# anhtu293/nndepth

Measured on AMD Instinct MI355X. Metric: stereo pairs/sec at 544x960, 32 iters (RAFT-Stereo), higher is better.
Workload: dtype f32 carried as 2 range-scaled fp16 pieces per operand (3 MFMA products, fp32 accumulate); 1 GPU; RAFT-Stereo base (ctx 64), 544x960, 32 iters, batch 1 per GPU, all 32 up_disp emitted; parallelism=single, launch=direct

## Files before the change

### nndepth_amd/csrc/common.h

```cpp
#pragma once
#include <hip/hip_runtime.h>
#include <atomic>
#include <cstdarg>
#include <cstdio>
#include "../../include/nndepth_amd.h"
#include "split_arith.h"

namespace nnd {

void set_error(const char* fmt, ...);

#define NND_HIP_CHECK(expr)                                                              \
    do {                                                                                 \
        hipError_t _e = (expr);                                                          \
        if (_e != hipSuccess) {                                                          \
            nnd::set_error("%s failed: %s (%s:%d)", #expr, hipGetErrorString(_e), __FILE__, __LINE__); \
            return NND_ERR_HIP;                                                          \
        }                                                                                \
    } while (0)

#define NND_LAUNCH_CHECK()                                                               \
    do {                                                                                 \
        hipError_t _e = hipGetLastError();                                               \
        if (_e != hipSuccess) {                                                          \
// ... 9 lines not shown
            return NND_ERR_INVALID;                                                      \
        }                                                                                \
    } while (0)

#define NND_TRY(x)                           \
    do {                                     \
        if ((rc = (x)) != NND_OK) return rc; \
    } while (0)

template <class Desc>
static inline int check_desc(const Desc* d, unsigned allowed_flags, const char* name) {
    NND_REQUIRE(d, "%s: null descriptor", name);
    NND_REQUIRE(d->struct_size == (int32_t)sizeof(Desc), "%s: descriptor of %d bytes, this library expects %d (struct_size)", name,
                d->struct_size, (int)sizeof(Desc));
    NND_REQUIRE((d->flags & ~allowed_flags) == 0, "%s: unknown flags 0x%x", name, d->flags);
    return NND_OK;
}

struct Switches {
    bool no_fused_upsample, no_fused_lookup, no_fused_flow_branch, no_c4, agcl_v1, no_thin3d, corr_build_v1, corr_build_no_ksplit, igev_squeeze_v1, igev_squeeze_walk, no_folded_flow_head, no_conv1x1_stream,
        conv_verbose, debug_sync;
    int split_ny, split_ks, split_p;
    bool split_no_fast;
    bool no_merged_fb_lookup;
    int conv_p, conv_ks, conv_wco;
    int agcl_pb;
    bool lds_poison_on;
    unsigned lds_poison;
    int lds_slack;
    bool enc_no_c4;
    bool no_slab3d;
    int slab3d_rounds;
    bool no_fused_enc_block;
};
const Switches& switches();

static inline int raise_lds_limit(const void* kern, std::atomic<unsigned>& done, int bytes = 160 * 1024) {
    int dev = 0;
    NND_HIP_CHECK(hipGetDevice(&dev));
    const unsigned bit = 1u << (dev & 31);
    if (!(done.load(std::memory_order_relaxed) & bit)) {
        NND_HIP_CHECK(hipFuncSetAttribute(kern, hipFuncAttributeMaxDynamicSharedMemorySize, bytes));
        done.fetch_or(bit, std::memory_order_relaxed);
    }
    return NND_OK;
}

bool calibrating();
struct CalibScope {
    explicit CalibScope(bool on);
    ~CalibScope();
    CalibScope(const CalibScope&) = delete;
    CalibScope& operator=(const CalibScope&) = delete;
    bool on;
};
struct Act;
struct Lay;
int calib_amax_act(const Act& a, const Lay& lay, int B, int H, int W, const float* tail, hipStream_t s);
int calib_amax_flat(const float* x, int64_t n, const float* tail, hipStream_t s);
int calib_finish(float* blob, const int64_t* tail_offs, int n, int32_t* status_dev, hipStream_t s);

#ifdef __HIPCC__
__device__ __forceinline__ void fmac_scalar(float& acc, float a, float b) { asm("v_fmac_f32 %0, %1, %2" : "+v"(acc) : "v"(a), "v"(b)); }

__device__ __forceinline__ float relu_nan(float v) { return __builtin_elementwise_maximum(v, 0.f); }
__device__ __forceinline__ float clamp_nan(float v, float lo, float hi) {
// ... 42 lines not shown
    int64_t bstride;
    int C;
};

struct ConvIO {
    Act src0, src1;
    Act out0, out1;
    Act aux0, aux1;
    Act bmap;
    int hidden = 0;
    float scale = 1.f;
    int Hin = 0, Win = 0;
    int flags = 0;
    bool src_tiled = false;
    bool dst_tiled = false;
    bool src_c4 = false;
    bool dst_c4 = false;
    int cout_need = 0;
    int force_ks = 0;
};

static inline bool conv_shape_built(int KH, int KW) { return (KH == 1 && (KW == 1 || KW == 5)) || (KW == 1 && KH == 5) || (KH == 3 && KW == 3); }

int conv_ci_t(int KH, int KW, int Cin, int stride = 1, int Cout = 0);

int launch_conv(const ConvLayer& L, const float* blob, const ConvIO& io, int epi,
                int B, int H, int W, hipStream_t stream);

void pack_conv(const ConvLayer& L, int nparts, const float* const* w, const float* const* b,
               const int* cout, float* blob, const int* ci_map = nullptr, int cin_src = 0);

bool conv_split_supported(int KH, int KW, int Cin, int stride, int arith, int Cout = 0);
int launch_conv_split(const ConvLayer& L, const float* blob, const ConvIO& io, int epi, int B, int H, int W, hipStream_t stream);
bool conv_split_no_split_k(const ConvLayer& L, int B, int H, int W);
bool flow_branch_supported(const ConvLayer& f2, int fc);
int launch_flow_branch(const ConvLayer& f2, const float* blob, const float* w7t, const float* b7, const float* flow, int64_t fbs,
                       int fc, const ConvIO& io, int B, int H, int W, hipStream_t stream);
void pack_conv_split(const ConvLayer& L, int nparts, const float* const* w, const float* const* b, const int* cout, float* blob,
                     const int* ci_map, int cin_src);

bool enc_block_supported(const ConvLayer& c1, const ConvLayer& c2, const ConvLayer& ds);
int enc_block_launch(const ConvLayer& c1, const float* blob1, const ConvLayer& c2, const float* blob2, const ConvLayer& ds, const float* blobd,
                     const float* x, float* out, int N, int Hx, int Wx, hipStream_t stream);

bool thin3d_supported(int Cout, int stride);
bool slab3d_supported(int Cout, int C0, int C1, int stride, int arith);
int64_t slab3d_packed_floats(int Cout, int Ct, int stride);
void slab3d_pack(int Cout, int Ct, int stride, const float* w, const float* scale, const float* shift, float* out);
int slab3d_forward(int Cout, int C0, int C1, int stride, const float* packed, const float* x0, const float* x1, float* y, int N, int D,
                   int H, int W, float slope, hipStream_t s);
int64_t thin3d_packed_floats(int Cout, int Ct);
void thin3d_pack(int Cout, int Ct, const float* w, const float* scale, const float* shift, float* out);
int thin3d_forward(int Cout, int C0, int C1, int stride, const float* packed, const float* x0, const float* x1, float* y, int N, int D,
                   int H, int W, float slope, hipStream_t s);

int corr1d_lookup_launch(const float* pyr, const float* coords, float* out, int B, int H, int W, int num_levels,
                         int radius, hipStream_t stream, bool tiled);
int group_lookup_flat_launch(const float* pyr, const float* coords, float* out, int B, int G, int H, int W, int num_levels, int radius,
                             hipStream_t stream, bool tiled);
int igev_lookup_launch(const float* feat_pyramid, const float* geo_pyramid, const float* coords, float* out, int B, int G, int H,
                       int W, int num_levels, int radius, hipStream_t stream, bool tiled);
int convex_upsample_launch(const float* flow, const float* mask, float* out, int B, int C, int H, int W, int rate,
                           hipStream_t stream, bool tiled);

int agcl_iter_launch(const float* f1, const float* f2, const float* flow, float* warped, float* out, int N, int C, int H,
                     int W, int small_patch, hipStream_t s, bool tiled);
// ... 38 lines not shown
```

### nndepth_amd/csrc/conv_split.hip

```cpp
#include "conv_launch.h"
#include "conv_split_kernel.h"
#include "flow_branch.h"

#include <atomic>
#include <cmath>
#include <cstdlib>
#include <cstring>

namespace nnd {

namespace {
uint16_t f16_rn(float x) {
    const _Float16 h = (_Float16)x;
    uint16_t u;
    memcpy(&u, &h, 2);
    return u;
}
float f16_to_f(uint16_t u) {
    _Float16 h;
    memcpy(&h, &u, 2);
    return (float)h;
}
uint16_t bf16_rn(float x) {
    uint32_t u;
// ... 85 lines not shown

bool restrict_split(const ConvLayer& L, int cout_need, SplitCfg* cfg) {
    const int npos = split_patch(L.KH, L.KW, L.arith, L.stride).NPOS;
    auto units = [&](int wco) { return split_staging_units(cfg->P, npos, cfg->ks, wco * cfg->ks); };
    if (!conv_restrict_cout(L, cout_need, &cfg->ny, &cfg->wco, [&](int wco) { return cfg->P == 2 && units(wco) <= 4; })) return false;
    cfg->nu = split_nu_variant(units(cfg->wco));
    return true;
}

bool split_fast_ok(const ConvLayer& L) { return !switches().split_no_fast || L.stride == 2; }
bool plan_split(const ConvLayer& L, const ConvIO& io, int B, int H, int W, SplitCfg* cfg) {
    if (!pick_split(L, io.src0.C, io.src1.C, B, H, W, split_fast_ok(L), cfg)) return false;
    cfg->restricted = restrict_split(L, io.cout_need, cfg);
    cfg->grid = dim3(cdiv(cfg->ntiles, cfg->P), cfg->ny, B), cfg->block = dim3(64 * cfg->wco * cfg->ks);
    return true;
}

void print_split_plan(const ConvLayer& L, const ConvIO& io, const SplitCfg& cfg) {
    fprintf(stderr, "[nnd] conv_split %dx%d Cin=%d Cout=%d pieces=%d: ny=%d, wco=%d, ks=%d, P=%d, nu=%d%s, grid %ux%ux%u, lds %zu B%s%s\n", L.KH,
            L.KW, L.Cin, L.Cout, L.arith, cfg.ny, cfg.wco, cfg.ks, cfg.P, cfg.nu, cfg.fast ? ", fast" : "", cfg.grid.x, cfg.grid.y, cfg.grid.z, cfg.lds,
            io.cout_need > 0 ? (cfg.restricted ? ", restricted to the wanted output channels" : ", whole layer (not restrictable)") : "",
            L.stride == 2 ? ", stride 2" : "");
}
}

bool conv_split_no_split_k(const ConvLayer& L, int B, int H, int W) {
    SplitCfg cfg;
    return pick_split(L, L.Cin, 0, B, H, W, split_fast_ok(L), &cfg) && cfg.ks == 1;
}

extern template int launch_split_ns<1>(const ConvArgs&, const SplitCfg&, int, int, hipStream_t);
extern template int launch_split_ns<2>(const ConvArgs&, const SplitCfg&, int, int, hipStream_t);
extern template int launch_split_ns<3>(const ConvArgs&, const SplitCfg&, int, int, hipStream_t);

bool conv_split_supported(int KH, int KW, int Cin, int stride, int arith, int Cout) {
    if ((arith != 3 && arith != 2 && arith != 1) || (stride != 1 && stride != 2) || Cin % 16 != 0) return false;
    if (stride == 2) return ((KH == 3 && KW == 3) || (KH == 1 && KW == 1)) && Cout >= 96;
    return conv_shape_built(KH, KW);
}

int launch_conv_split(const ConvLayer& L, const float* blob, const ConvIO& io, int epi, int B, int H, int W, hipStream_t stream) {
    int rc, Hin, Win;
    NND_REQUIRE(conv_split_supported(L.KH, L.KW, L.Cin, L.stride, L.arith, L.Cout), "conv_split: %dx%d Cin=%d Cout=%d stride %d arith %d not built",
                L.KH, L.KW, L.Cin, L.Cout, L.stride, L.arith);
    NND_TRY(conv_check_io("conv_split", L, io, epi, H, W, &Hin, &Win));
    NND_REQUIRE(L.CI_T == 16 && L.nchunks * 16 == L.Cin, "conv_split: layer was not planned for 16-channel chunks");
    NND_REQUIRE(L.stride == 1 || io.src1.C == 0, "conv_split: stride 2 is built for one source");
    NND_REQUIRE((long)(L.Cin + 64) * tiled_plane(Hin, Win) < (1L << 31), "conv_split: plane offsets exceed 32 bits");
    SplitCfg cfg;
    NND_REQUIRE(plan_split(L, io, B, H, W, &cfg),
                "conv_split: no configuration for %dx%d Cin=%d (%d+%d) Cout=%d stride %d (NND_SPLIT_CFG ny=%d ks=%d P=%d%s)", L.KH, L.KW,
                L.Cin, io.src0.C, io.src1.C, L.Cout, L.stride, switches().split_ny, switches().split_ks, switches().split_p,
                split_fast_ok(L) ? "" : ", NND_SPLIT_NO_FAST");
    ConvArgs a;
    conv_fill_args(L, blob, io, epi, H, W, Hin, Win, &a);
    a.tiles_x = cfg.tiles_x; a.wco = cfg.wco; a.ks = cfg.ks; a.npos = cfg.ntiles;
#ifdef NND_DBG_STAMPS
    {
        static std::atomic<int> launches{0};
        static const int only = getenv("NND_DBG_STAMP_LAUNCH") ? atoi(getenv("NND_DBG_STAMP_LAUNCH")) : -1;
        const int idx = launches.fetch_add(1);
        a.dbg_stamp = only < 0 || idx == only;
    }
#endif
    if (calibrating() && split_range_scaled(L.arith))
        for (const Act* src : {&io.src0, &io.src1}) NND_TRY(calib_amax_act(*src, a.ls, B, Hin, Win, blob + L.tail_off(), stream));
    if (switches().conv_verbose) print_split_plan(L, io, cfg);
    rc = L.arith == 3   ? launch_split_ns<3>(a, cfg, L.KH, L.KW, stream)
         : L.arith == 2 ? launch_split_ns<2>(a, cfg, L.KH, L.KW, stream)
                        : launch_split_ns<1>(a, cfg, L.KH, L.KW, stream);
    NND_REQUIRE(rc != NND_ERR_UNSUPPORTED, "conv_split: shape %dx%d P=%d nu=%d %s is not instantiated", L.KH, L.KW, cfg.P, cfg.nu, cfg.fast ? "fast" : "generic");
    if (rc != NND_OK) return rc;
    NND_LAUNCH_CHECK();
    return NND_OK;
}

void pack_conv_split(const ConvLayer& L, int nparts, const float* const* w, const float* const* bvec, const int* cout, float* blob,
                     const int* ci_map, int cin_src) {
    if (!ci_map) cin_src = L.Cin;
    const int NT = L.KH * L.KW, NS = L.arith;
    uint16_t* wp = reinterpret_cast<uint16_t*>(blob + L.w_off);
    float* bp = blob + L.b_off;
    memset(wp, 0, sizeof(float) * L.w_floats());
    memset(bp, 0, sizeof(float) * L.b_floats());
    const bool f16 = split_range_scaled(NS);
    float wscale = 1.f;
    if (f16) {
        float wmax = 0.f;
        for (int part = 0; part < nparts; ++part)
            for (int col = 0; col < cout[part]; ++col)
                for (int ci = 0; ci < L.Cin; ++ci)
                    for (int t = 0; t < NT; ++t) {
                        const float v = std::fabs(w[part][((size_t)col * cin_src + (ci_map ? ci_map[ci] : ci)) * NT + t]);
                        if (std::isfinite(v) && v > wmax) wmax = v;
                    }
        int e = 0;
        if (wmax > 0.f) std::frexp(wmax, &e);
        const int s = wmax > 0.f ? 14 - e : 0;
        wscale = std::ldexp(1.f, s);
        float* tail = bp + L.ncb * 32;
        tail[SPLIT_TAIL_OSCALE] = std::ldexp(1.f, -(s + SPLIT_F16_XSHIFT));
        tail[SPLIT_TAIL_XSCALE] = std::ldexp(1.f, SPLIT_F16_XSHIFT);
        tail[SPLIT_TAIL_AMAX] = 0.f;
        tail[SPLIT_TAIL_WSINV] = std::ldexp(1.f, -s);
// ... 76 lines not shown
```

### nndepth_amd/csrc/conv_split_kernel.h

```cpp
#pragma once
#include "common.h"
#include "conv_epilogue.h"
#include "layout.h"
#include "split_arith.h"

#include <type_traits>
#include <utility>

namespace nnd {

#ifndef NND_SPLIT_BSLOTS
#define NND_SPLIT_BSLOTS 2
#endif

#ifdef NND_DBG_STAMPS
static __device__ unsigned long long g_split_stamps[4096 * 8];
#define NND_SSTAMP(i)                                                                                  \
    do {                                                                                               \
        if (threadIdx.x == 0 && a.dbg_stamp) {                                                         \
            const unsigned lin_ = blockIdx.x + gridDim.x * (blockIdx.y + gridDim.y * blockIdx.z);      \
            if (lin_ < 4096) g_split_stamps[lin_ * 8 + (i)] = __builtin_amdgcn_s_memrealtime();        \
        }                                                                                              \
    } while (0)
#define NND_SCLOCK(i)                                                                                  \
// ... 42 lines not shown
struct SplitPatch {
    int PRI, PCI, NPH, PRP, PCP, NPOS, PS, ROWB, PHB, SUBB;
};
__host__ __device__ constexpr SplitPatch split_patch(int KH, int KW, int NS, int STR) {
    const int PRI = 3 * STR + KH, PCI = 7 * STR + KW;
    const int NPH = STR == 1 ? 1 : (KH * KW == 1 ? 1 : 4);
    const int PRP = STR == 1 ? PRI : (KH == 1 ? 4 : (PRI + 1) / 2);
    const int PCP = STR == 1 ? PCI : (KW == 1 ? 8 : (PCI + 1) / 2);
    const int NPOS = STR == 1 ? PRI * PCI : (KH * KW == 1 ? 32 : PRI * PCI);
    const int ROWB = split_row_bytes(PCP, NS);
    return {PRI, PCI, NPH, PRP, PCP, NPOS, split_pos_bytes(NS), ROWB, PRP * ROWB, NPH * PRP * ROWB};
}
template <int KH, int KW, int NS, int STR>
struct SplitGeom {
    static constexpr SplitPatch G = split_patch(KH, KW, NS, STR);
    static constexpr int PRI = G.PRI, PCI = G.PCI, NPH = G.NPH, PRP = G.PRP, PCP = G.PCP, NPOS = G.NPOS;
    static constexpr int PS = G.PS, ROWB = G.ROWB, PHB = G.PHB, SUBB = G.SUBB;
};
__host__ __device__ constexpr int split_staging_units(int P, int npos, int ks, int waves) { return (P * npos * 2 * ks + 64 * waves - 1) / (64 * waves); }
__host__ __device__ constexpr int split_nu_variant(int nu) { return nu <= 2 ? 2 : 4; }

__host__ __device__ constexpr int split_pipe_spu(int nunit, int nsteps, int ul) {
    int v = 1;
    while (v < nsteps && nunit - 1 - (nsteps + v - 1) / v < ul + 3) ++v;
    return v;
}
template <int NT, int P, int NU>
struct SplitPipe {
    static constexpr int NUNIT = NT * P, NSTEPS = NU * 4 + 3, UL = 1;
    static constexpr int SPU = split_pipe_spu(NUNIT, NSTEPS, UL), U0 = NUNIT - 1 - (NSTEPS + SPU - 1) / SPU;
    static constexpr bool ON = NT >= 5 && P == 2;
};

template <int KH, int KW, int NS, int P, int NU, bool FAST, bool SRC4, int AD_, int MAXT, int STR = 1>
__global__ void __launch_bounds__(MAXT) conv_split_kernel(ConvArgs a) {
    static_assert(STR == 1 || (FAST && (KH * KW == 9 || KH * KW == 1)), "stride 2: 3x3 / 1x1, FAST regime");
    using Geo = SplitGeom<KH, KW, NS, STR>;
    constexpr int NT = KH * KW, PH = KH / 2, PW = KW / 2;
    constexpr int PC = Geo::PCI, NPOS = Geo::NPOS;
#ifndef NND_SPLIT_NO_PIPE
    constexpr bool PIPE = FAST && SRC4 && SplitPipe<NT, P, NU>::ON && NS != 1;
#else
    constexpr bool PIPE = false;
#endif
    constexpr int PS = Geo::PS, ROWB = Geo::ROWB, SUBB = Geo::SUBB, PHB = Geo::PHB;
    extern __shared__ __attribute__((aligned(16))) unsigned char lds_raw[];
    NND_SSTAMP(0);

    const int tid = threadIdx.x, lane = tid & 63, nthreads = blockDim.x;
    const int wave = __builtin_amdgcn_readfirstlane(tid >> 6);
    const int wco = a.wco, ks = a.ks;
    const int cbi = wave % wco, kj = wave / wco;
    const int h2 = lane >> 5, l31 = lane & 31;
    const int pxl = lane_pixel(l31), r = pxl >> 3, c = pxl & 7;
    const int cb = blockIdx.y * wco + cbi;
    const bool active = cb * 32 < a.Cout;
    const int b = blockIdx.z;
    const int Hin = a.Hin, Win = a.Win;
    const long SP = a.ls.plane;
    const int SCH = ks * 16;
    float oscale = 1.f, xscale = 1.f;
    if constexpr (split_range_scaled(NS)) {
        const float* tail = a.bias + (((a.Cout + 31) >> 5) << 5);
        oscale = tail[SPLIT_TAIL_OSCALE];
        xscale = tail[SPLIT_TAIL_XSCALE];
    }

    int ty0[P], tx0[P];
#pragma unroll
    for (int pp = 0; pp < P; ++pp) {
        const int t = blockIdx.x * P + pp;
        const bool valid = t < a.npos;
        ty0[pp] = valid ? (t / a.tiles_x) * 4 : (1 << 20);
        tx0[pp] = valid ? (t % a.tiles_x) * 8 : 0;
    }

    const int nunits = P * NPOS * 2 * ks;
    int goff[NU], loff[NU], cho[NU];
    bool inimg[NU], own[NU];
#pragma unroll
    for (int i = 0; i < NU; ++i) {
        const int u = PIPE ? min(tid + i * nthreads, nunits - 1) : tid + i * nthreads;
        own[i] = u < nunits;
        const int pos = u % NPOS, rest = u / NPOS;
        const int pp = rest % P, oct = rest / P;
        int pr, pc, lpos;
        if constexpr (STR == 1) {
            pr = pos / PC;
// ... 447 lines not shown
}

template <int KH, int KW, int NS, bool FAST, bool SRC4, int STR>
int launch_split_nu(const ConvArgs& a, const SplitCfg& cfg, hipStream_t stream) {
    constexpr int AD = FAST ? split_fast_ad<KH, KW, NS>() : 1;
    if (split_nu_variant(cfg.nu) == 2) return launch_split_kernel<KH, KW, NS, 2, 2, FAST, SRC4, AD, 768, STR>(a, cfg.grid, cfg.block, cfg.lds, stream);
    return launch_split_kernel<KH, KW, NS, 2, 4, FAST, SRC4, AD, 768, STR>(a, cfg.grid, cfg.block, cfg.lds, stream);
}
template <int KH, int KW, int NS>
int launch_split_shape(const ConvArgs& a, const SplitCfg& cfg, hipStream_t stream) {
    if (cfg.P != 2) return NND_ERR_UNSUPPORTED;
    const bool src4 = a.ls.ci == 4;
    if (cfg.stride == 2) {
        if constexpr (KH * KW == 9 || KH * KW == 1) {
            if (!cfg.fast) return NND_ERR_UNSUPPORTED;
            return src4 ? launch_split_nu<KH, KW, NS, true, true, 2>(a, cfg, stream) : launch_split_nu<KH, KW, NS, true, false, 2>(a, cfg, stream);
        } else {
            return NND_ERR_UNSUPPORTED;
        }
    }
    if (!cfg.fast) return launch_split_nu<KH, KW, NS, false, false, 1>(a, cfg, stream);
    return src4 ? launch_split_nu<KH, KW, NS, true, true, 1>(a, cfg, stream) : launch_split_nu<KH, KW, NS, true, false, 1>(a, cfg, stream);
}

template <int NS>
int launch_split_ns(const ConvArgs& a, const SplitCfg& cfg, int KH, int KW, hipStream_t stream) {
    if (KH == 3 && KW == 3) return launch_split_shape<3, 3, NS>(a, cfg, stream);
    if (KH == 1 && KW == 5) return launch_split_shape<1, 5, NS>(a, cfg, stream);
    if (KH == 5 && KW == 1) return launch_split_shape<5, 1, NS>(a, cfg, stream);
    if (KH == 1 && KW == 1) return launch_split_shape<1, 1, NS>(a, cfg, stream);
    return NND_ERR_UNSUPPORTED;
}

}
```

### nndepth_amd/csrc/conv_split_ns1.hip

```cpp
#include "conv_split_kernel.h"

namespace nnd {
template int launch_split_ns<1>(const ConvArgs&, const SplitCfg&, int, int, hipStream_t);
#ifdef NND_DBG_STAMPS
extern "C" int nnd_debug_read_split_stamps_ns1(unsigned long long* host, int n) {
    return hipMemcpyFromSymbol(host, HIP_SYMBOL(g_split_stamps), sizeof(unsigned long long) * n) == hipSuccess ? 0 : -1;
}
#endif
}
```

### nndepth_amd/csrc/conv_split_ns2.hip

```cpp
#include "conv_split_kernel.h"

namespace nnd {
template int launch_split_ns<2>(const ConvArgs&, const SplitCfg&, int, int, hipStream_t);
#ifdef NND_DBG_STAMPS
extern "C" int nnd_debug_read_split_stamps_ns2(unsigned long long* host, int n) {
    return hipMemcpyFromSymbol(host, HIP_SYMBOL(g_split_stamps), sizeof(unsigned long long) * n) == hipSuccess ? 0 : -1;
}
#endif
}
```

### nndepth_amd/csrc/conv_split_ns3.hip

```cpp
#include "conv_split_kernel.h"

namespace nnd {
template int launch_split_ns<3>(const ConvArgs&, const SplitCfg&, int, int, hipStream_t);
#ifdef NND_DBG_STAMPS
extern "C" int nnd_debug_read_split_stamps_ns3(unsigned long long* host, int n) {
    return hipMemcpyFromSymbol(host, HIP_SYMBOL(g_split_stamps), sizeof(unsigned long long) * n) == hipSuccess ? 0 : -1;
}
#endif
}
```

### nndepth_amd/csrc/error.cpp

```cpp
#include "common.h"

#include <cstdlib>

namespace nnd {
static thread_local char g_err[512] = "";
void set_error(const char* fmt, ...) {
    va_list ap;
    va_start(ap, fmt);
    vsnprintf(g_err, sizeof(g_err), fmt, ap);
    va_end(ap);
}

static Switches g_sw;
static void load_switches() {
    Switches s{};
    auto on = [](const char* n) { return getenv(n) != nullptr; };
    s.no_fused_upsample = on("NND_NO_FUSED_UPSAMPLE");
    s.no_fused_lookup = on("NND_NO_FUSED_LOOKUP");
    s.no_fused_flow_branch = on("NND_NO_FUSED_FLOW_BRANCH");
    s.no_c4 = on("NND_NO_C4");
    s.agcl_v1 = on("NND_AGCL_V1");
    s.no_thin3d = on("NND_NO_THIN3D");
    s.corr_build_v1 = on("NND_CORR_BUILD_V1");
    s.corr_build_no_ksplit = on("NND_CORR_BUILD_NO_KSPLIT");
    s.igev_squeeze_v1 = on("NND_IGEV_SQUEEZE_V1");
    s.igev_squeeze_walk = on("NND_IGEV_SQUEEZE_WALK");
    s.no_folded_flow_head = on("NND_NO_FOLDED_FLOW_HEAD");
    s.no_conv1x1_stream = on("NND_NO_CONV1X1_STREAM");
    s.conv_verbose = on("NND_CONV_VERBOSE");
    s.debug_sync = on("NND_DEBUG_SYNC");
    s.split_ny = s.split_ks = s.split_p = -1;
    if (const char* e = getenv("NND_SPLIT_CFG")) sscanf(e, "%d,%d,%d", &s.split_ny, &s.split_ks, &s.split_p);
    s.split_no_fast = on("NND_SPLIT_NO_FAST");
    s.no_merged_fb_lookup = on("NND_NO_MERGED_FB_LOOKUP");
    s.conv_p = s.conv_ks = s.conv_wco = -1;
    if (const char* e = getenv("NND_CONV_CFG")) sscanf(e, "%d,%d,%d", &s.conv_p, &s.conv_ks, &s.conv_wco);
    if (const char* e = getenv("NND_CONV_P")) s.conv_p = atoi(e);
    s.agcl_pb = getenv("NND_AGCL_PB") ? atoi(getenv("NND_AGCL_PB")) : 0;
    s.lds_poison_on = on("NND_DEBUG_LDS_POISON");
    s.lds_poison = s.lds_poison_on ? (unsigned)strtoul(getenv("NND_DEBUG_LDS_POISON"), nullptr, 0) : 0u;
    s.lds_slack = getenv("NND_DEBUG_LDS_SLACK") ? atoi(getenv("NND_DEBUG_LDS_SLACK")) : 0;
    s.enc_no_c4 = on("NND_ENC_NO_C4");
    s.no_slab3d = on("NND_NO_SLAB3D");
    s.slab3d_rounds = getenv("NND_SLAB3D_ROUNDS") ? atoi(getenv("NND_SLAB3D_ROUNDS")) : 0;
    s.no_fused_enc_block = on("NND_NO_FUSED_ENC_BLOCK");
    g_sw = s;
}
namespace {
struct SwitchInit {
    SwitchInit() { load_switches(); }
} g_switch_init;
}
const Switches& switches() { return g_sw; }
}

extern "C" {
int nnd_reload_switches(void) {
    nnd::load_switches();
    return NND_OK;
}
int nnd_version(void) { return NND_VERSION; }
const char* nnd_last_error(void) { return nnd::g_err; }
int nnd_device_count(void) {
    int n = 0;
    if (hipGetDeviceCount(&n) != hipSuccess) {
        (void)hipGetLastError();
        return 0;
    }
    return n;
}
}
```

### nndepth_amd/csrc/update_block.hip

```cpp
#include "common.h"
#include "conv_layer.h"
#include "layout.h"

#include <cstdlib>
#include <cstring>
#include <vector>

namespace nnd {

enum ConvId { C_C1 = 0, C_C2, C_F2, C_CV, C_ZR1X, C_Q1X, C_ZR2X, C_Q2X, C_FHM, C_M2, C_LOOP_COUNT,
              C_ZR1 = C_LOOP_COUNT, C_Q1, C_ZR2, C_Q2, C_ZR1C, C_Q1C, C_ZR2C, C_Q2C, C_COUNT };
static const char* kConvNames[C_COUNT] = {"encoder.convc1", "encoder.convc2", "encoder.convf2", "encoder.conv",
                                          "gru.convz1+convr1[h,motion]", "gru.convq1[rh,motion]", "gru.convz2+convr2[h,motion]",
                                          "gru.convq2[rh,motion]", "flow_head.conv1+mask.0", "mask.2",
                                          "gru.convz1+convr1", "gru.convq1", "gru.convz2+convr2", "gru.convq2",
                                          "gru.convz1+convr1[inp]", "gru.convq1[inp]", "gru.convz2+convr2[inp]", "gru.convq2[inp]"};

struct Plan {
    nnd_update_block_desc d;
    bool sep;
    int num_tensors;
    ConvLayer L[C_COUNT];
    int64_t f1_w, f1_b;
    int64_t f1_wt;
// ... 135 lines not shown
__global__ void init_coords_kernel(float* __restrict__ coords, float* __restrict__ flow, float* __restrict__ hx_flow,
                                   long hx_bs, int hx_pm, const float* __restrict__ disp_init, int B, int H, int W, int absolute, Lay lay) {
    const long HW = (long)H * W;
    long idx = (long)blockIdx.x * blockDim.x + threadIdx.x;
    if (idx >= B * HW) return;
    const int b = (int)(idx / HW);
    const long pix = idx % HW;
    const int x = (int)(pix % W);
    const long po = pix_off(lay, (int)(pix / W), x);
    float c = (float)x + (disp_init ? disp_init[idx] : 0.f);
    float f = absolute ? c : c - (float)x;
    coords[b * lay.plane + po] = c;
    flow[b * lay.plane + po] = f;
    hx_flow[b * hx_bs + po * hx_pm] = f;
}

__global__ void to_tiled_kernel(const float* __restrict__ src, float* __restrict__ dst, long dbs, int c0, int B, int C, int H, int W, Lay lay) {
    const long HW = (long)H * W;
    long idx = (long)blockIdx.x * blockDim.x + threadIdx.x;
    if (idx >= (long)B * C * HW) return;
    const long pix = idx % HW;
    const int c = (int)((idx / HW) % C), b = (int)(idx / (HW * C));
    dst[b * dbs + chan_off(lay, c0 + c) + pix_off(lay, (int)(pix / W), (int)(pix % W))] = src ? src[idx] : 0.f;
}
__global__ void from_tiled_kernel(const float* __restrict__ src, long sbs, int c0, float* __restrict__ dst, int B, int C, int H, int W, Lay lay) {
    const long HW = (long)H * W;
    long idx = (long)blockIdx.x * blockDim.x + threadIdx.x;
    if (idx >= (long)B * C * HW) return;
    const long pix = idx % HW;
    const int c = (int)((idx / HW) % C), b = (int)(idx / (HW * C));
    dst[idx] = src[b * sbs + chan_off(lay, c0 + c) + pix_off(lay, (int)(pix / W), (int)(pix % W))];
}

template <int FC>
__global__ void __launch_bounds__(512) flow_head2_kernel(const float* __restrict__ x, long xbs, int hid, const float* __restrict__ w,
                                                         const float* __restrict__ bias, float* __restrict__ delta,
                                                         float* __restrict__ coords, float* __restrict__ flow,
                                                         float* __restrict__ hx_flow, long hx_bs, int hx_cs, int hx_pm, int x_c4, int H,
                                                         int W, int tiles_x, int advance, int absolute, Lay lay) {
    extern __shared__ float sm[];
    float* patch = sm;
    float* wl = sm + hid * 64;
    float* part = wl + FC * hid * 9;
    const int tid = threadIdx.x;
    const int tx0 = (blockIdx.x % tiles_x) * 8, ty0 = (blockIdx.x / tiles_x) * 4, b = blockIdx.z;
    const long HW = lay.plane;
    const float* src = x + b * xbs;
    float tail_bias = 0.f, tail_state = 0.f;
    if (tid < 32 * FC) {
        const int f = tid >> 5, p2 = tid & 31;
        const int y = ty0 + (p2 >> 3), xx = tx0 + (p2 & 7);
        tail_bias = bias[f];
        if (y < H && xx < W) {
            const long pix = pix_off(lay, y, xx);
            if (advance == 2) tail_state = flow[(b * FC + f) * HW + pix];
            else if (advance) tail_state = coords[b * HW + pix];
        }
    }
    {
        const int pos = tid & 63, cg = tid >> 6;
        const int gy = ty0 + pos / 10 - 1, gx = tx0 + pos % 10 - 1;
        const bool ok = pos < 60 && gy >= 0 && gy < H && gx >= 0 && gx < W;
        const long off = ok ? pix_off(lay, gy, gx) : 0;
        if (x_c4) {
            for (int q0 = cg; q0 < hid / 4; q0 += 32) {
                float4 v4[4];
// ... 482 lines not shown
                          const CreArgs* cre = nullptr, const float* interleaved = nullptr, int flat_groups = 0) {
    Plan p;
    int rc = make_plan(desc, &p);
    if (rc != NND_OK) return rc;
    const bool last_flag = (p.d.flags & NND_FLAG_LAST_UPSAMPLE_ONLY) != 0;
    NND_REQUIRE(!last_flag || up_iter_stride == 0,
                "refine: NND_FLAG_LAST_UPSAMPLE_ONLY writes one upsampled map, so up_iter_stride must be 0 (got %lld)", (long long)up_iter_stride);
    const bool last_only = last_flag && !(p.d.flags & NND_FLAG_CALIBRATE);
    NND_REQUIRE(packed && (pyramid || cre) && net && inp && up_out && workspace, "refine: null pointer");
    const bool igev = geo_pyramid != nullptr;
    const int fc = p.d.flow_channels;
    if (cre) {
        NND_REQUIRE(fc == 2 && p.d.cor_planes == 36, "cre_stereo_refine: needs flow_channels 2 and cor_planes 36");
        NND_REQUIRE(cre->f1 && cre->f2 && (cre->extra || cre->warped), "cre_stereo_refine: null feature map / scratch");
        NND_REQUIRE(cre->extra || cre->warped_floats >= (int64_t)B * cre->C * H * W,
                    "cre_stereo_refine: iter mode needs a scratch of B*C*H*W = %lld floats, got %lld", (long long)B * cre->C * H * W,
                    (long long)cre->warped_floats);
    } else {
        NND_REQUIRE(fc == 1, "raft_stereo_refine: flow_channels must be 1");
        NND_REQUIRE(p.d.cor_planes == num_levels * (2 * radius + 1) * (igev ? 2 * groups : (flat_groups > 0 ? flat_groups : 1)),
                    "refine: cor_planes %d does not match levels*(2r+1)%s", p.d.cor_planes, igev ? "*2*groups" : (flat_groups > 0 ? "*groups" : ""));
        NND_REQUIRE(!(igev && flat_groups > 0), "refine: the IGEV and the group-RAFT lookups exclude each other");
    }

    NND_REQUIRE(p.d.mask_channels == 9 * rate * rate, "raft_stereo_refine: mask_channels %d != 9*rate^2", p.d.mask_channels);
    NND_REQUIRE(B > 0 && H > 0 && W > 0 && iters > 0, "raft_stereo_refine: bad shape");
    CalibScope calib((p.d.flags & NND_FLAG_CALIBRATE) && split_range_scaled(p.d.arithmetic));
    hipStream_t s = (hipStream_t)stream;
    Bufs w;
    carve(p, B, H, W, workspace, &w);
    const int hid = p.d.hidden_dim, ctx = p.d.context_dim, hxC = 2 * hid + ctx;
    const Lay lay = make_lay(H, W, true);
    const int64_t n = lay.plane;
    NND_TRY(to_tiled(net, w.hx, hxC * n, B, hid, H, W, s, 0, ws_c4()));
    NND_TRY(to_tiled(inp, w.hx, hxC * n, B, ctx, H, W, s, hid, ws_c4()));
    float* hx_flow = w.hx + ws_chan(hxC - fc, n);
    const unsigned eg = (unsigned)cdiv64((int64_t)B * H * W, 256);
    if (cre) {
        if (disp_init) {
            NND_TRY(to_tiled(disp_init, w.flow, fc * n, B, fc, H, W, s));
            NND_TRY(to_tiled(disp_init, w.hx, hxC * n, B, fc, H, W, s, hxC - fc, ws_c4()));
        } else {
            NND_HIP_CHECK(hipMemsetAsync(w.flow, 0, sizeof(float) * B * fc * n, s));
            NND_TRY(to_tiled(nullptr, w.hx, hxC * n, B, fc, H, W, s, hxC - fc, ws_c4()));
        }
    } else {
        hipLaunchKernelGGL(init_coords_kernel, dim3(eg), dim3(256), 0, s, w.coords, w.flow, hx_flow, (long)(hxC * n), ws_pm(), disp_init, B, H,
                           W, igev ? 1 : 0, lay);
        NND_LAUNCH_CHECK();
    }
    const bool cre_cl = cre && cre->extra && cre->warped && cre->warped_floats >= 2 * (int64_t)B * cre->C * H * W &&
                        agcl_offset_cl_supported(cre->C) && !switches().agcl_v1;
    if (cre_cl) {
        NND_TRY(nchw_to_nhwc_launch(cre->f1, cre->warped, B, cre->C, H * W, s));
        NND_TRY(nchw_to_nhwc_launch(cre->f2, cre->warped + (int64_t)B * cre->C * H * W, B, cre->C, H * W, s));
    }
    Act c = act(w.corr, p.d.cor_planes * n, p.d.cor_planes);
    auto lookup = [&](hipStream_t st_, int it) -> int {
        if (cre) {
            if (cre->extra && cre_cl)
                return agcl_offset_cl_launch(cre->warped, cre->warped + (int64_t)B * cre->C * H * W, w.flow, cre->extra, w.corr, B, cre->C,
                                             H, W, it & 1, st_, true);
            if (cre->extra) return agcl_offset_launch(cre->f1, cre->f2, w.flow, cre->extra, w.corr, B, cre->C, H, W, it & 1, st_, true);
            return agcl_iter_launch(cre->f1, cre->f2, w.flow, cre->warped, w.corr, B, cre->C, H, W, it & 1, st_, true);
        }
        if (igev) return igev_lookup_launch(pyramid, geo_pyramid, w.coords, w.corr, B, groups, H, W, num_levels, radius, st_, true);
        if (flat_groups > 0) return group_lookup_flat_launch(pyramid, w.coords, w.corr, B, flat_groups, H, W, num_levels, radius, st_, true);
        return corr1d_lookup_launch(pyramid, w.coords, w.corr, B, H, W, num_levels, radius, st_, true);
    };
    for (int id : {(int)C_ZR1C, (int)C_Q1C, (int)C_ZR2C, (int)C_Q2C})
        if (p.sep || id < C_ZR2C) NND_TRY(run_conv(p, packed, w, id, c, nullptr, nullptr, B, H, W, s));
    const bool no_fuse_up = switches().no_fused_upsample;
    const bool no_fuse_lk = switches().no_fused_lookup;
    const bool fused_up = !no_fuse_up && mask_upsample_supported(rate, 2 * hid, fc);
    const bool fold_fh = fused_up && !cre && fc == 1 && mask_upsample_fold_supported(p.L[C_M2], hid) &&
                         (long)B * cdiv(H, 4) * cdiv(W, 8) <= 256 && !switches().no_folded_flow_head;
    float* coords_alt = w.mask;
    float* flow_alt = w.mask + ((int64_t)B * n + 63) / 64 * 64;
    const bool fused_lk = !cre && !no_fuse_lk && flat_groups == 0;
    const bool merged_fbl = fused_lk && !igev && !switches().no_merged_fb_lookup && !switches().no_fused_flow_branch &&
                            flow_branch_supported(p.L[C_F2], fc) && flow_branch_lookup_supported(p.L[C_F2].arith);
    auto loop_conv = [&](int id) -> int {
        probe_mark(id, s);
        const int rc_ = run_conv(p, packed, w, id, c, nullptr, nullptr, B, H, W, s);
        probe_mark(id, s);
        return rc_;
    };
    if (calibrating() && fused_lk && interleaved && p.L[C_C1].range_scaled() && igev_lookup_convc1_il_supported(groups, num_levels, radius))
        NND_TRY(calib_amax_flat(interleaved, nnd_igev_interleaved_floats(B, groups, H, W, num_levels), packed + p.L[C_C1].tail_off(), s));
    for (int it = 0; it < iters; ++it) {
        if (merged_fbl) {
            probe_mark(C_F2, s);
            NND_TRY(calib_flow_branch(p, packed, w, w.flow, B, H, W, s));
            const ConvIO fio = conv_io(p, w, C_F2, c, n, nullptr, nullptr);
            NND_TRY(flow_branch_lookup_launch(p.L[C_F2], packed, packed + p.f1_wt, packed + p.f1_b, w.flow, (int64_t)fc * n, fc, fio, pyramid,
                                              w.coords, p.L[C_C1], w.c1, 256 * n, B, H, W, num_levels, radius, s, ws_c4()));
            NND_TRY(debug_sync("encoder.convf1+convf2 | lookup+convc1", s));
            probe_mark(C_F2, s);
        } else {
        probe_mark(C_F2, s);
        NND_TRY(run_flow_branch(p, packed, w, w.flow, c, B, H, W, s));
        probe_mark(C_F2, s);
        if (fused_lk && interleaved && igev_lookup_convc1_il_supported(groups, num_levels, radius)) {
            NND_TRY(igev_lookup_convc1_il_launch(interleaved, groups, w.coords, p.L[C_C1], packed, w.c1, 256 * n, B, H, W, num_levels,
// ... 21 lines not shown
            ConvIO io = conv_io(p, w, C_FHM, c, n, nullptr, nullptr);
            io.cout_need = hid;
            NND_TRY(launch_conv(p.L[C_FHM], packed, io, conv_epi(C_FHM), B, H, W, s));
            NND_TRY(debug_sync("flow_head.conv1", s));
            NND_TRY(run_fc2(p, packed, w, w.delta, cre ? 2 : 1, igev, B, H, W, s));
            continue;
        }
        NND_TRY(loop_conv(C_FHM));
        float* up_it = up_out + (int64_t)it * up_iter_stride;
        if (fold_fh) {
            MaskUpFlowHead fh;
            fh.x = w.fm; fh.xbs = (int64_t)3 * hid * n; fh.hid = hid;
            fh.w = packed + p.fc2_w; fh.bias = packed + p.fc2_b;
            fh.coords_in = w.coords; fh.coords_out = coords_alt; fh.flow_out = flow_alt; fh.delta_out = w.delta;
            fh.hx_flow = hx_flow; fh.hx_bs = (long)(hxC * n); fh.hx_pm = ws_pm(); fh.absolute = igev ? 1 : 0;
            NND_TRY(mask_upsample_launch(p.L[C_M2], packed, w.fm + hid * n, (int64_t)3 * hid * n, w.flow, up_it, B, H, W, rate, s,
                                         true, fc, ws_c4(), &fh));
            NND_TRY(debug_sync("flow_head.conv2 + mask.2 + upsample", s));
            std::swap(w.coords, coords_alt);
            std::swap(w.flow, flow_alt);
            continue;
        }
        NND_TRY(run_fc2(p, packed, w, w.delta, cre ? 2 : 1, igev, B, H, W, s));
        if (fused_up) {
            NND_TRY(mask_upsample_launch(p.L[C_M2], packed, w.fm + hid * n, (int64_t)3 * hid * n, w.flow, up_it, B, H, W, rate, s,
                                         true, fc, ws_c4()));
            NND_TRY(debug_sync("mask.2 + upsample", s));
        } else {
            NND_TRY(run_conv(p, packed, w, C_M2, c, w.mask, nullptr, B, H, W, s));
            NND_TRY(convex_upsample_launch(w.flow, w.mask, up_it, B, fc, H, W, rate, s, true));
            NND_TRY(debug_sync("convex upsample", s));
        }
    }
    if (low_out) NND_TRY(from_tiled(w.flow, fc * n, low_out, B, fc, H, W, s));
    if (net_out) NND_TRY(from_tiled(w.hx, hxC * n, net_out, B, hid, H, W, s, 0, ws_c4()));
    return NND_OK;
}

static int conv2d_layer(int Cout, int Cin, int KH, int KW, int arithmetic, ConvLayer* L, int64_t* total) {
    NND_REQUIRE(Cout > 0 && Cin > 0, "conv2d: bad channel counts");
    NND_REQUIRE(conv_shape_built(KH, KW), "conv2d: kernel %dx%d not built (1x1, 3x3, 1x5, 5x1)", KH, KW);
    NND_REQUIRE(arithmetic == 0 || conv_split_supported(KH, KW, Cin, 1, arithmetic),
                "conv2d: arithmetic %d not built for %dx%d with %d input channels (3 = bf16x3, 2 = fp16x2, 1 = fp16: Cin %% 16 == 0)", arithmetic, KH, KW, Cin);
    int64_t off = 0;
    *L = mk(KH, KW, Cin, Cout, &off, arithmetic);
    if (total) *total = off;
    return NND_OK;
}

int64_t nnd_conv2d_packed_floats_ex(int Cout, int Cin, int KH, int KW, int arithmetic) {
    ConvLayer L;
    int64_t total;
    if (conv2d_layer(Cout, Cin, KH, KW, arithmetic, &L, &total) != NND_OK) return NND_ERR_INVALID;
    return total;
}
int64_t nnd_conv2d_packed_floats(int Cout, int Cin, int KH, int KW) { return nnd_conv2d_packed_floats_ex(Cout, Cin, KH, KW, 0); }

int nnd_conv2d_pack_ex(const float* w_host, const float* b_host, int Cout, int Cin, int KH, int KW, int arithmetic, float* packed_host) {
    ConvLayer L;
    int rc = conv2d_layer(Cout, Cin, KH, KW, arithmetic, &L, nullptr);
    if (rc != NND_OK) return rc;
    NND_REQUIRE(w_host && b_host && packed_host, "conv2d_pack: null pointer");
    const float* w[1] = {w_host};
    const float* b[1] = {b_host};
    int co[1] = {Cout};
    pack_conv(L, 1, w, b, co, packed_host);
// ... 320 lines not shown
```

Before: 149.7 pairs/s.

## Group paired context convs into one launch and merge loop entry/exit copies

Adds a grouped conv_split kernel variant that runs two same-shape convolutions (the zr and q context convs) in one launch by splitting blockIdx.y between the two layers' argument sets. It also merges the loop-entry copies (net and inp to tiled layout, plus coords/flow initialization) into one kernel, and the loop-exit from_tiled copies into one kernel. The intent is to cut kernel launch count and small-kernel tail overhead outside the 32-iteration loop. The grouped path falls back to two launches when the plans differ. Both paths can be turned off with switches.

Result: no change. 150.1 pairs/s, median of 6 (+0.3%).

```diff
diff --git a/nndepth_amd/csrc/common.h b/nndepth_amd/csrc/common.h
--- a/nndepth_amd/csrc/common.h
+++ b/nndepth_amd/csrc/common.h
@@ -65,6 +65,8 @@
     bool no_slab3d;
     int slab3d_rounds;
     bool no_fused_enc_block;
+    bool no_grouped_ctx;
+    bool no_merged_loop_io;
 };
 const Switches& switches();
 
@@ -173,6 +175,8 @@
 
 bool conv_split_supported(int KH, int KW, int Cin, int stride, int arith, int Cout = 0);
 int launch_conv_split(const ConvLayer& L, const float* blob, const ConvIO& io, int epi, int B, int H, int W, hipStream_t stream);
+int launch_conv_pair(const ConvLayer& L0, const ConvIO& io0, int epi0, const ConvLayer& L1, const ConvIO& io1, int epi1, const float* blob,
+                     int B, int H, int W, hipStream_t stream);
 bool conv_split_no_split_k(const ConvLayer& L, int B, int H, int W);
 bool flow_branch_supported(const ConvLayer& f2, int fc);
 int launch_flow_branch(const ConvLayer& f2, const float* blob, const float* w7t, const float* b7, const float* flow, int64_t fbs,
diff --git a/nndepth_amd/csrc/conv_split.hip b/nndepth_amd/csrc/conv_split.hip
--- a/nndepth_amd/csrc/conv_split.hip
+++ b/nndepth_amd/csrc/conv_split.hip
@@ -141,6 +141,9 @@
 extern template int launch_split_ns<1>(const ConvArgs&, const SplitCfg&, int, int, hipStream_t);
 extern template int launch_split_ns<2>(const ConvArgs&, const SplitCfg&, int, int, hipStream_t);
 extern template int launch_split_ns<3>(const ConvArgs&, const SplitCfg&, int, int, hipStream_t);
+extern template int launch_split_pair_ns<1>(const ConvPairArgs&, const SplitCfg&, int, int, hipStream_t);
+extern template int launch_split_pair_ns<2>(const ConvPairArgs&, const SplitCfg&, int, int, hipStream_t);
+extern template int launch_split_pair_ns<3>(const ConvPairArgs&, const SplitCfg&, int, int, hipStream_t);
 
 bool conv_split_supported(int KH, int KW, int Cin, int stride, int arith, int Cout) {
     if ((arith != 3 && arith != 2 && arith != 1) || (stride != 1 && stride != 2) || Cin % 16 != 0) return false;
@@ -148,7 +151,8 @@
     return conv_shape_built(KH, KW);
 }
 
-int launch_conv_split(const ConvLayer& L, const float* blob, const ConvIO& io, int epi, int B, int H, int W, hipStream_t stream) {
+static int prepare_split(const ConvLayer& L, const float* blob, const ConvIO& io, int epi, int B, int H, int W, ConvArgs* args, SplitCfg* plan,
+                         int* Hin_out, int* Win_out) {
     int rc, Hin, Win;
     NND_REQUIRE(conv_split_supported(L.KH, L.KW, L.Cin, L.stride, L.arith, L.Cout), "conv_split: %dx%d Cin=%d Cout=%d stride %d arith %d not built",
                 L.KH, L.KW, L.Cin, L.Cout, L.stride, L.arith);
@@ -156,14 +160,23 @@
     NND_REQUIRE(L.CI_T == 16 && L.nchunks * 16 == L.Cin, "conv_split: layer was not planned for 16-channel chunks");
     NND_REQUIRE(L.stride == 1 || io.src1.C == 0, "conv_split: stride 2 is built for one source");
     NND_REQUIRE((long)(L.Cin + 64) * tiled_plane(Hin, Win) < (1L << 31), "conv_split: plane offsets exceed 32 bits");
-    SplitCfg cfg;
+    SplitCfg& cfg = *plan;
     NND_REQUIRE(plan_split(L, io, B, H, W, &cfg),
                 "conv_split: no configuration for %dx%d Cin=%d (%d+%d) Cout=%d stride %d (NND_SPLIT_CFG ny=%d ks=%d P=%d%s)", L.KH, L.KW,
                 L.Cin, io.src0.C, io.src1.C, L.Cout, L.stride, switches().split_ny, switches().split_ks, switches().split_p,
                 split_fast_ok(L) ? "" : ", NND_SPLIT_NO_FAST");
-    ConvArgs a;
+    ConvArgs& a = *args;
     conv_fill_args(L, blob, io, epi, H, W, Hin, Win, &a);
     a.tiles_x = cfg.tiles_x; a.wco = cfg.wco; a.ks = cfg.ks; a.npos = cfg.ntiles;
+    *Hin_out = Hin, *Win_out = Win;
+    return NND_OK;
+}
+
+int launch_conv_split(const ConvLayer& L, const float* blob, const ConvIO& io, int epi, int B, int H, int W, hipStream_t stream) {
+    int rc, Hin, Win;
+    SplitCfg cfg;
+    ConvArgs a;
+    NND_TRY(prepare_split(L, blob, io, epi, B, H, W, &a, &cfg, &Hin, &Win));
 #ifdef NND_DBG_STAMPS
     {
         static std::atomic<int> launches{0};
@@ -179,6 +192,41 @@
          : L.arith == 2 ? launch_split_ns<2>(a, cfg, L.KH, L.KW, stream)
                         : launch_split_ns<1>(a, cfg, L.KH, L.KW, stream);
     NND_REQUIRE(rc != NND_ERR_UNSUPPORTED, "conv_split: shape %dx%d P=%d nu=%d %s is not instantiated", L.KH, L.KW, cfg.P, cfg.nu, cfg.fast ? "fast" : "generic");
+    if (rc != NND_OK) return rc;
+    NND_LAUNCH_CHECK();
+    return NND_OK;
+}
+
+int launch_conv_pair(const ConvLayer& L0, const ConvIO& io0, int epi0, const ConvLayer& L1, const ConvIO& io1, int epi1, const float* blob,
+                     int B, int H, int W, hipStream_t stream) {
+    int rc;
+    auto two = [&]() -> int {
+        NND_TRY(launch_conv(L0, blob, io0, epi0, B, H, W, stream));
+        return launch_conv(L1, blob, io1, epi1, B, H, W, stream);
+    };
+    if (calibrating() || L0.arith == 0 || L1.arith != L0.arith || L0.KH != L1.KH || L0.KW != L1.KW || L0.stride != 1 || L1.stride != 1) return two();
+    int Hin, Win;
+    SplitCfg c0, c1;
+    ConvPairArgs g;
+    memset(&g, 0, sizeof(g));
+    NND_TRY(prepare_split(L0, blob, io0, epi0, B, H, W, &g.l[0], &c0, &Hin, &Win));
+    NND_TRY(prepare_split(L1, blob, io1, epi1, B, H, W, &g.l[1], &c1, &Hin, &Win));
+    const bool same = c0.wco == c1.wco && c0.ks == c1.ks && c0.P == c1.P && split_nu_variant(c0.nu) == split_nu_variant(c1.nu) && c0.fast == c1.fast &&
+                      c0.lds == c1.lds && c0.stride == c1.stride && c0.grid.x == c1.grid.x && c0.grid.z == c1.grid.z && c0.block.x == c1.block.x &&
+                      g.l[0].ls.ci == g.l[1].ls.ci;
+    if (!same || !split_pair_built(L0.KH, L0.KW, c0, g.l[0].ls.ci == 4) || (long)c0.grid.y + c1.grid.y > 65535) return two();
+    if (switches().conv_verbose) {
+        print_split_plan(L0, io0, c0);
+        print_split_plan(L1, io1, c1);
+        fprintf(stderr, "[nnd] conv_split: the two layers above as one grouped launch, grid %ux%ux%u\n", c0.grid.x, c0.grid.y + c1.grid.y, c0.grid.z);
+    }
+    g.ny0 = (int)c0.grid.y;
+    SplitCfg cfg = c0;
+    cfg.grid.y = c0.grid.y + c1.grid.y;
+    rc = L0.arith == 3   ? launch_split_pair_ns<3>(g, cfg, L0.KH, L0.KW, stream)
+         : L0.arith == 2 ? launch_split_pair_ns<2>(g, cfg, L0.KH, L0.KW, stream)
+                         : launch_split_pair_ns<1>(g, cfg, L0.KH, L0.KW, stream);
+    NND_REQUIRE(rc != NND_ERR_UNSUPPORTED, "conv_split: grouped shape %dx%d nu=%d is not instantiated", L0.KH, L0.KW, cfg.nu);
     if (rc != NND_OK) return rc;
     NND_LAUNCH_CHECK();
     return NND_OK;
diff --git a/nndepth_amd/csrc/conv_split_kernel.h b/nndepth_amd/csrc/conv_split_kernel.h
--- a/nndepth_amd/csrc/conv_split_kernel.h
+++ b/nndepth_amd/csrc/conv_split_kernel.h
@@ -98,8 +98,22 @@
     static constexpr bool ON = NT >= 5 && P == 2;
 };
 
-template <int KH, int KW, int NS, int P, int NU, bool FAST, bool SRC4, int AD_, int MAXT, int STR = 1>
-__global__ void __launch_bounds__(MAXT) conv_split_kernel(ConvArgs a) {
+struct ConvPairArgs {
+    ConvArgs l[2];
+    int ny0;
+};
+__device__ __forceinline__ const ConvArgs& split_layer_args(const ConvArgs& g, int&) { return g; }
+__device__ __forceinline__ const ConvArgs& split_layer_args(const ConvPairArgs& g, int& by) {
+    const bool second = by >= g.ny0;
+    by -= second ? g.ny0 : 0;
+    return second ? g.l[1] : g.l[0];
+}
+
+template <int KH, int KW, int NS, int P, int NU, bool FAST, bool SRC4, int AD_, int MAXT, int STR = 1, bool PAIR = false>
+__global__ void __launch_bounds__(MAXT) conv_split_kernel(std::conditional_t<PAIR, ConvPairArgs, ConvArgs> g) {
+    int by_ = (int)blockIdx.y;
+    const ConvArgs& a = split_layer_args(g, by_);
+    const int by = by_;
     static_assert(STR == 1 || (FAST && (KH * KW == 9 || KH * KW == 1)), "stride 2: 3x3 / 1x1, FAST regime");
     using Geo = SplitGeom<KH, KW, NS, STR>;
     constexpr int NT = KH * KW, PH = KH / 2, PW = KW / 2;
@@ -119,7 +133,7 @@
     const int cbi = wave % wco, kj = wave / wco;
     const int h2 = lane >> 5, l31 = lane & 31;
     const int pxl = lane_pixel(l31), r = pxl >> 3, c = pxl & 7;
-    const int cb = blockIdx.y * wco + cbi;
+    const int cb = by * wco + cbi;
     const bool active = cb * 32 < a.Cout;
     const int b = blockIdx.z;
     const int Hin = a.Hin, Win = a.Win;
@@ -633,4 +647,33 @@
     return NND_ERR_UNSUPPORTED;
 }
 
-}
+template <int KH, int KW, int NS, int NU>
+int launch_split_pair_kernel(const ConvPairArgs& g, const SplitCfg& cfg, hipStream_t stream) {
+    constexpr int AD = split_fast_ad<KH, KW, NS>();
+    auto kern = conv_split_kernel<KH, KW, NS, 2, NU, true, true, AD, 768, 1, true>;
+    if ((int)cfg.block.x > 768) return NND_ERR_UNSUPPORTED;
+    const size_t lds = cfg.lds + switches().lds_slack;
+    if (lds > 64 * 1024) {
+        static std::atomic<unsigned> raised{0};
+        if (int rc = raise_lds_limit(reinterpret_cast<const void*>(kern), raised)) return rc;
+    }
+    hipLaunchKernelGGL(kern, cfg.grid, cfg.block, lds, stream, g);
+    return NND_OK;
+}
+template <int KH, int KW, int NS>
+int launch_split_pair_shape(const ConvPairArgs& g, const SplitCfg& cfg, hipStream_t stream) {
+    if (split_nu_variant(cfg.nu) == 2) return launch_split_pair_kernel<KH, KW, NS, 2>(g, cfg, stream);
+    return launch_split_pair_kernel<KH, KW, NS, 4>(g, cfg, stream);
+}
+inline bool split_pair_built(int KH, int KW, const SplitCfg& cfg, bool src4) {
+    return ((KH == 3 && KW == 3) || (KH == 1 && KW == 5) || (KH == 5 && KW == 1)) && cfg.stride == 1 && cfg.P == 2 && cfg.fast && src4;
+}
+template <int NS>
+int launch_split_pair_ns(const ConvPairArgs& g, const SplitCfg& cfg, int KH, int KW, hipStream_t stream) {
+    if (!split_pair_built(KH, KW, cfg, g.l[0].ls.ci == 4 && g.l[1].ls.ci == 4)) return NND_ERR_UNSUPPORTED;
+    if (KH == 3 && KW == 3) return launch_split_pair_shape<3, 3, NS>(g, cfg, stream);
+    if (KH == 1 && KW == 5) return launch_split_pair_shape<1, 5, NS>(g, cfg, stream);
+    return launch_split_pair_shape<5, 1, NS>(g, cfg, stream);
+}
+
+}
diff --git a/nndepth_amd/csrc/conv_split_ns1.hip b/nndepth_amd/csrc/conv_split_ns1.hip
--- a/nndepth_amd/csrc/conv_split_ns1.hip
+++ b/nndepth_amd/csrc/conv_split_ns1.hip
@@ -2,6 +2,7 @@
 
 namespace nnd {
 template int launch_split_ns<1>(const ConvArgs&, const SplitCfg&, int, int, hipStream_t);
+template int launch_split_pair_ns<1>(const ConvPairArgs&, const SplitCfg&, int, int, hipStream_t);
 #ifdef NND_DBG_STAMPS
 extern "C" int nnd_debug_read_split_stamps_ns1(unsigned long long* host, int n) {
     return hipMemcpyFromSymbol(host, HIP_SYMBOL(g_split_stamps), sizeof(unsigned long long) * n) == hipSuccess ? 0 : -1;
diff --git a/nndepth_amd/csrc/conv_split_ns2.hip b/nndepth_amd/csrc/conv_split_ns2.hip
--- a/nndepth_amd/csrc/conv_split_ns2.hip
+++ b/nndepth_amd/csrc/conv_split_ns2.hip
@@ -2,6 +2,7 @@
 
 namespace nnd {
 template int launch_split_ns<2>(const ConvArgs&, const SplitCfg&, int, int, hipStream_t);
+template int launch_split_pair_ns<2>(const ConvPairArgs&, const SplitCfg&, int, int, hipStream_t);
 #ifdef NND_DBG_STAMPS
 extern "C" int nnd_debug_read_split_stamps_ns2(unsigned long long* host, int n) {
     return hipMemcpyFromSymbol(host, HIP_SYMBOL(g_split_stamps), sizeof(unsigned long long) * n) == hipSuccess ? 0 : -1;
diff --git a/nndepth_amd/csrc/conv_split_ns3.hip b/nndepth_amd/csrc/conv_split_ns3.hip
--- a/nndepth_amd/csrc/conv_split_ns3.hip
+++ b/nndepth_amd/csrc/conv_split_ns3.hip
@@ -2,6 +2,7 @@
 
 namespace nnd {
 template int launch_split_ns<3>(const ConvArgs&, const SplitCfg&, int, int, hipStream_t);
+template int launch_split_pair_ns<3>(const ConvPairArgs&, const SplitCfg&, int, int, hipStream_t);
 #ifdef NND_DBG_STAMPS
 extern "C" int nnd_debug_read_split_stamps_ns3(unsigned long long* host, int n) {
     return hipMemcpyFromSymbol(host, HIP_SYMBOL(g_split_stamps), sizeof(unsigned long long) * n) == hipSuccess ? 0 : -1;
diff --git a/nndepth_amd/csrc/error.cpp b/nndepth_amd/csrc/error.cpp
--- a/nndepth_amd/csrc/error.cpp
+++ b/nndepth_amd/csrc/error.cpp
@@ -44,6 +44,8 @@
     s.no_slab3d = on("NND_NO_SLAB3D");
     s.slab3d_rounds = getenv("NND_SLAB3D_ROUNDS") ? atoi(getenv("NND_SLAB3D_ROUNDS")) : 0;
     s.no_fused_enc_block = on("NND_NO_FUSED_ENC_BLOCK");
+    s.no_grouped_ctx = on("NND_NO_GROUPED_CTX");
+    s.no_merged_loop_io = on("NND_NO_MERGED_LOOP_IO");
     g_sw = s;
 }
 namespace {
diff --git a/nndepth_amd/csrc/update_block.hip b/nndepth_amd/csrc/update_block.hip
--- a/nndepth_amd/csrc/update_block.hip
+++ b/nndepth_amd/csrc/update_block.hip
@@ -191,6 +191,49 @@
     dst[idx] = src[b * sbs + chan_off(lay, c0 + c) + pix_off(lay, (int)(pix / W), (int)(pix % W))];
 }
 
+__global__ void loop_entry_kernel(const float* __restrict__ net, const float* __restrict__ inp, float* __restrict__ hx, long hx_bs, int hid,
+                                  int ctx, Lay hlay, float* __restrict__ coords, float* __restrict__ flow, float* __restrict__ hx_flow,
+                                  int hx_pm, const float* __restrict__ disp_init, int absolute, Lay lay, int B, int H, int W) {
+    const long HW = (long)H * W;
+    const int C = hid + ctx;
+    long idx = (long)blockIdx.x * blockDim.x + threadIdx.x;
+    const long ncopy = (long)B * C * HW;
+    if (idx < ncopy) {
+        const long pix = idx % HW;
+        const int c = (int)((idx / HW) % C), b = (int)(idx / (HW * C));
+        const float v = c < hid ? net[((long)b * hid + c) * HW + pix] : inp[((long)b * ctx + (c - hid)) * HW + pix];
+        hx[b * hx_bs + chan_off(hlay, c) + pix_off(hlay, (int)(pix / W), (int)(pix % W))] = v;
+        return;
+    }
+    idx -= ncopy;
+    if (!coords || idx >= B * HW) return;
+    const int b = (int)(idx / HW);
+    const long pix = idx % HW;
+    const int x = (int)(pix % W);
+    const long po = pix_off(lay, (int)(pix / W), x);
+    float c = (float)x + (disp_init ? disp_init[idx] : 0.f);
+    float f = absolute ? c : c - (float)x;
+    coords[b * lay.plane + po] = c;
+    flow[b * lay.plane + po] = f;
+    hx_flow[b * hx_bs + po * hx_pm] = f;
+}
+
+__global__ void loop_exit_kernel(const float* __restrict__ hx, long hx_bs, int hid, Lay hlay, float* __restrict__ net_out,
+                                 const float* __restrict__ flow, long flow_bs, int fc, Lay lay, float* __restrict__ low_out, int B, int H, int W) {
+    const long HW = (long)H * W;
+    long idx = (long)blockIdx.x * blockDim.x + threadIdx.x;
+    const long nnet = (long)B * hid * HW;
+    const bool second = idx >= nnet;
+    if (second) idx -= nnet;
+    const int C = second ? fc : hid;
+    if (idx >= (long)B * C * HW) return;
+    const long pix = idx % HW;
+    const int c = (int)((idx / HW) % C), b = (int)(idx / (HW * C));
+    const int y = (int)(pix / W), x = (int)(pix % W);
+    if (second) low_out[idx] = flow[b * flow_bs + chan_off(lay, c) + pix_off(lay, y, x)];
+    else net_out[idx] = hx[b * hx_bs + chan_off(hlay, c) + pix_off(hlay, y, x)];
+}
+
 template <int FC>
 __global__ void __launch_bounds__(512) flow_head2_kernel(const float* __restrict__ x, long xbs, int hid, const float* __restrict__ w,
                                                          const float* __restrict__ bias, float* __restrict__ delta,
@@ -739,10 +782,18 @@
     const int hid = p.d.hidden_dim, ctx = p.d.context_dim, hxC = 2 * hid + ctx;
     const Lay lay = make_lay(H, W, true);
     const int64_t n = lay.plane;
-    NND_TRY(to_tiled(net, w.hx, hxC * n, B, hid, H, W, s, 0, ws_c4()));
-    NND_TRY(to_tiled(inp, w.hx, hxC * n, B, ctx, H, W, s, hid, ws_c4()));
     float* hx_flow = w.hx + ws_chan(hxC - fc, n);
     const unsigned eg = (unsigned)cdiv64((int64_t)B * H * W, 256);
+    const bool merged_io = !switches().no_merged_loop_io;
+    if (merged_io) {
+        const int64_t elems = (int64_t)B * (hid + ctx) * H * W + (cre ? 0 : (int64_t)B * H * W);
+        hipLaunchKernelGGL(loop_entry_kernel, dim3((unsigned)cdiv64(elems, 256)), dim3(256), 0, s, net, inp, w.hx, (long)(hxC * n), hid, ctx,
+                           make_lay(H, W, true, ws_c4()), cre ? nullptr : w.coords, w.flow, hx_flow, ws_pm(), disp_init, igev ? 1 : 0, lay, B, H, W);
+        NND_LAUNCH_CHECK();
+    } else {
+        NND_TRY(to_tiled(net, w.hx, hxC * n, B, hid, H, W, s, 0, ws_c4()));
+        NND_TRY(to_tiled(inp, w.hx, hxC * n, B, ctx, H, W, s, hid, ws_c4()));
+    }
     if (cre) {
         if (disp_init) {
             NND_TRY(to_tiled(disp_init, w.flow, fc * n, B, fc, H, W, s));
@@ -751,7 +802,7 @@
             NND_HIP_CHECK(hipMemsetAsync(w.flow, 0, sizeof(float) * B * fc * n, s));
             NND_TRY(to_tiled(nullptr, w.hx, hxC * n, B, fc, H, W, s, hxC - fc, ws_c4()));
         }
-    } else {
+    } else if (!merged_io) {
         hipLaunchKernelGGL(init_coords_kernel, dim3(eg), dim3(256), 0, s, w.coords, w.flow, hx_flow, (long)(hxC * n), ws_pm(), disp_init, B, H,
                            W, igev ? 1 : 0, lay);
         NND_LAUNCH_CHECK();
@@ -775,8 +826,18 @@
         if (flat_groups > 0) return group_lookup_flat_launch(pyramid, w.coords, w.corr, B, flat_groups, H, W, num_levels, radius, st_, true);
         return corr1d_lookup_launch(pyramid, w.coords, w.corr, B, H, W, num_levels, radius, st_, true);
     };
-    for (int id : {(int)C_ZR1C, (int)C_Q1C, (int)C_ZR2C, (int)C_Q2C})
-        if (p.sep || id < C_ZR2C) NND_TRY(run_conv(p, packed, w, id, c, nullptr, nullptr, B, H, W, s));
+    for (int zr : {(int)C_ZR1C, (int)C_ZR2C}) {
+        if (!p.sep && zr == C_ZR2C) continue;
+        const int q = zr + 1;
+        if (switches().no_grouped_ctx) {
+            NND_TRY(run_conv(p, packed, w, zr, c, nullptr, nullptr, B, H, W, s));
+            NND_TRY(run_conv(p, packed, w, q, c, nullptr, nullptr, B, H, W, s));
+            continue;
+        }
+        const ConvIO io_zr = conv_io(p, w, zr, c, n, nullptr, nullptr), io_q = conv_io(p, w, q, c, n, nullptr, nullptr);
+        NND_TRY(launch_conv_pair(p.L[zr], io_zr, conv_epi(zr), p.L[q], io_q, conv_epi(q), packed, B, H, W, s));
+        NND_TRY(debug_sync(kConvNames[zr], s));
+    }
     const bool no_fuse_up = switches().no_fused_upsample;
     const bool no_fuse_lk = switches().no_fused_lookup;
     const bool fused_up = !no_fuse_up && mask_upsample_supported(rate, 2 * hid, fc);
@@ -864,6 +925,13 @@
             NND_TRY(debug_sync("convex upsample", s));
         }
     }
+    if (low_out && net_out && merged_io) {
+        const int64_t elems = (int64_t)B * (hid + fc) * H * W;
+        hipLaunchKernelGGL(loop_exit_kernel, dim3((unsigned)cdiv64(elems, 256)), dim3(256), 0, s, w.hx, (long)(hxC * n), hid,
+                           make_lay(H, W, true, ws_c4()), net_out, w.flow, (long)(fc * n), fc, lay, low_out, B, H, W);
+        NND_LAUNCH_CHECK();
+        return NND_OK;
+    }
     if (low_out) NND_TRY(from_tiled(w.flow, fc * n, low_out, B, fc, H, W, s));
     if (net_out) NND_TRY(from_tiled(w.hx, hxC * n, net_out, B, hid, H, W, s, 0, ws_c4()));
     return NND_OK;
```
